# afombravo/2FAST2Q

Hardware: AMD Instinct MI355X
Metric: Mreads/sec matched (150 bp, 20 bp feature, m=1) (higher is better)
Workload: dtype u64 (2-bit packed bases) / u8 qualities

## Files before the change

2fast2q_amd/csrc/f2q_count_kernels.h:

```cpp
#pragma once

#define F2Q_HIST_MAX 24576u
#define F2Q_HIST_RANGE 38912u

__device__ __forceinline__ unsigned long long wave_sum(unsigned long long v)
{
    for (int o = 32; o > 0; o >>= 1) v += __shfl_down(v, o, 64);
    return v;
}

__device__ __forceinline__ void flush_stats(const Accum &acc, unsigned long long st[5], unsigned long long *lds8,
                                            unsigned long long *slab_row)
{
    const uint32_t lane = threadIdx.x & 63u;
    if (threadIdx.x < 8) lds8[threadIdx.x] = 0;
    __syncthreads();
    for (int k = 0; k < 5; k++) {
        unsigned long long v = wave_sum(st[k]);
        if (lane == 0 && v) atomicAdd(&lds8[k], v);
    }
    __syncthreads();
    if (threadIdx.x < 5) {
        unsigned long long v = lds8[threadIdx.x];
        if (slab_row) gpw(slab_row)[threadIdx.x] = v;
// ... 332 lines not shown
                    for (int r = 0; r < F2Q_MAXQROWS; r++)
                        if (r < g.nq) fixed4_qrow(g, r, qrow[r], bad);
                }
#pragma unroll
                for (int j = 0; j < 4; j++) {
                    if (res[j] != R_NEAR || bad[j]) continue;
                    key[j] |= fixed4_key(g, brow, j) << (2u * (uint32_t)L * npart[j]);
                    if (lv[j] & F2Q_LEN_FLAG) forced[j] |= fixed4_flags(g, qrow, j) << ((uint32_t)L * npart[j]);
                    npart[j]++;
                }
            }
#pragma unroll
            for (int j = 0; j < 4; j++) {
                if (res[j] == R_SLOW) {
                    unsigned long long st2[5] = {0, 0, 0, 0, 0};
                    const Accum acc2 = acc; const PackedBlock pb2 = pb;
                    multi_slow(runp, libp, &acc2, &pb2, tile, 4u * lane + (uint32_t)j, (int)(lv[j] & F2Q_LEN_MASK), st2);
#pragma unroll
                    for (int k = 0; k < 5; k++) st[k] += st2[k];
                    res[j] = R_SKIP;
                } else if (res[j] == R_NEAR) {
                    st[0]++;
                    if (npart[j] == 0u) { res[j] = R_QFAIL; st[4]++; }
                    else if (forced[j]) res[j] = (!do_near || __popc(forced[j]) > run.miss) ? R_NONALIGNED : R_FORCED;
                }
            }
            for (int k = W; k >= 1; k--) {
                bool mine[4]; bool any = false;
#pragma unroll
                for (int j = 0; j < 4; j++) { mine[j] = res[j] == R_NEAR && npart[j] == (uint32_t)k; any |= mine[j]; }
                if (__ballot(any) == 0ull) continue;
                const PackedGroup &pk = lib.mpk[k - 1];
                const PackedPiece ex = pk.exact;
                const uint32_t ib = pk.ib, exm = (1u << ex.bits) - 1u;
                const uint64_t imask = (1ull << ib) - 1ull;
                if (pk.len == 0u) continue;
                uint32_t s[4];
#pragma unroll
                for (int j = 0; j < 4; j++) s[j] = packed_start(key[j], ex.bits);
                while (mine[0] | mine[1] | mine[2] | mine[3]) {
                    uint64_t v0[4], v1[4];
#pragma unroll
                    for (int j = 0; j < 4; j++)
                        if (mine[j]) { const Slot2 pr = packed_pair(ptab, ex.off + s[j]); v0[j] = pr.a; v1[j] = pr.b; }
#pragma unroll
                    for (int j = 0; j < 4; j++) {
                        if (!mine[j]) continue;
                        if (v0[j] == KEY_EMPTY) mine[j] = false;
                        else if ((v0[j] >> ib) == key[j]) { mine[j] = false; res[j] = R_PERFECT; count_hit((uint32_t)(v0[j] & imask)); }
                        else if (v1[j] == KEY_EMPTY) mine[j] = false;
                        else if ((v1[j] >> ib) == key[j]) { mine[j] = false; res[j] = R_PERFECT; count_hit((uint32_t)(v1[j] & imask)); }
                        else s[j] = (s[j] + 2u) & exm;
                    }
                }
            }
            uint32_t npush = 0;
#pragma unroll
            for (int j = 0; j < 4; j++) {
                if (res[j] == R_NEAR) { if (do_near) npush++; else res[j] = R_NONALIGNED; }
                else if (res[j] == R_FORCED) npush++;
                st[1] += (res[j] == R_PERFECT); st[3] += (res[j] == R_NONALIGNED);
            }
            {
                const unsigned long long b0 = __ballot(npush & 1u), b1 = __ballot(npush & 2u), b2 = __ballot(npush & 4u);
                uint32_t at = q_tail + __builtin_amdgcn_mbcnt_hi((uint32_t)(b0 >> 32), __builtin_amdgcn_mbcnt_lo((uint32_t)b0, 0u))
                              + 2u * __builtin_amdgcn_mbcnt_hi((uint32_t)(b1 >> 32), __builtin_amdgcn_mbcnt_lo((uint32_t)b1, 0u))
                              + 4u * __builtin_amdgcn_mbcnt_hi((uint32_t)(b2 >> 32), __builtin_amdgcn_mbcnt_lo((uint32_t)b2, 0u));
                q_tail += (uint32_t)__popcll(b0) + 2u * (uint32_t)__popcll(b1) + 4u * (uint32_t)__popcll(b2);
#pragma unroll
                for (int j = 0; j < 4; j++)
                    if (res[j] == R_NEAR || res[j] == R_FORCED) {
                        queue[at % F2Q_V2_QCAP] = key[j] | ((unsigned long long)(npart[j] - 1u) << 62);
                        qforced[at % F2Q_V2_QCAP] = forced[j];
                        at++;
                    }
            }
        }
        if (do_near) drain(false);
    }
    if (do_near) drain(true);
    __shared__ unsigned long long st_lds[8];
    flush_stats(acc, st, st_lds, acc.stat_slab ? acc.stat_slab + (uint64_t)blockIdx.x * 8u : nullptr);
    if (USE_LDS) {
        __syncthreads();
        auto row = gpw(acc.slab) + (uint64_t)blockIdx.x * nf;
        for (uint32_t i = tid; i < nf; i += F2Q_V2_THREADS) row[i] = hist[i];
    }
}

#define F2Q_LT_THREADS 1024
#define F2Q_LT_WAVES (F2Q_LT_THREADS / 64)

__device__ __forceinline__ U2 lds_u2(const uint32_t *p)
{
    typedef uint32_t v2 __attribute__((ext_vector_type(2)));
    const v2 v = *reinterpret_cast<const v2 *>(p);
    return U2{v.x, v.y};
}

__device__ __forceinline__ uint32_t lt_count_add(uint32_t *cnt, uint32_t slot)
{
    return atomicAdd(&cnt[slot >> 1], 1u << ((slot & 1u) << 4));
}
__device__ __forceinline__ bool lt_count_passed(uint32_t old, uint32_t slot) { return ((old >> ((slot & 1u) << 4)) & 0xFFFFu) == 0x7FFFu; }
__device__ __forceinline__ void lt_count_handoff(uint32_t *cnt, uint32_t slot, const Accum &acc, const LtDesc &lt)
{
    atomicSub(&cnt[slot >> 1], 0x8000u << ((slot & 1u) << 4));
    acc_add(&acc.counts[gp(lt.feat_of)[slot]], 0x8000ull);
}
__device__ __forceinline__ void lt_count(uint32_t *cnt, uint32_t slot, const Accum &acc, const LtDesc &lt)
{
    if (lt_count_passed(lt_count_add(cnt, slot), slot)) lt_count_handoff(cnt, slot, acc, lt);
}

template <int NQ, int NB, bool NEAR, bool A20, bool MW = false>
__global__ __launch_bounds__(F2Q_LT_THREADS) void k_count_fixed4_lds(const RunDev *__restrict__ runp,
                                                                     const LibDev *__restrict__ libp, PackedBlock pb,
                                                                     Accum acc)
{
    extern __shared__ uint32_t lt_smem[];
    constexpr uint32_t NT = NEAR ? 2u : 1u;
    uint32_t *tg = lt_smem;
    uint32_t *cnt = lt_smem + NT * F2Q_LT_SLOTS;
    const RunDev &run = *runp;
    const LibDev &lib = *libp;
    LtDesc lt = lib.lt;
    if (A20) { lt.hb0 = 20u; lt.hb1 = 20u; lt.len = 20u; }
    const uint32_t nf = lib.n_features;
    const uint32_t tid = threadIdx.x, lane = tid & 63u;
    const uint32_t wave = (uint32_t)__builtin_amdgcn_readfirstlane((int)(tid >> 6));
    FixedGeom g = MW ? fixed_geom_at(0, run.n_iter * run.length, run.thr) : fixed_geom(run);
    if (A20) { g.L = 20; g.nq = 5; g.nb = 2; g.sh = 0; g.qm_first = 0x80808080u; g.qm_last = 0x80808080u; g.kmask = (1ull << 40) - 1ull; }
    const int need = g.st + g.L;
    uint32_t w_reads = 0, w_perfect = 0, w_imperfect = 0, w_qfail = 0;
    constexpr int QR = NQ ? NQ : F2Q_MAXQROWS, BR = NB ? NB : F2Q_MAXBROWS;
    constexpr bool PIPE = NQ != 0;

    struct Rows { U4 b[BR], q[QR]; uint32_t len01, len23; };
    const uint64_t q_stride = (uint64_t)pb.wq * F2Q_TILE, b_stride = (uint64_t)pb.wb * F2Q_TILE;
    const auto q_base = gp(pb.qual) + (uint64_t)g.qw0 * F2Q_TILE + 4u * lane;
    const auto b_base = gp(pb.bases) + (uint64_t)g.bw0 * F2Q_TILE + 4u * lane;
    const auto l_base = gp(pb.len) + 4u * lane;
    auto request_tile = [&](Rows &r, uint32_t t) {
        const auto qp = q_base + (uint64_t)t * q_stride;
        const auto bp = b_base + (uint64_t)t * b_stride;
#pragma unroll
        for (int i = 0; i < BR; i++) r.b[i] = ld_u4<true>(bp + (NB ? i : (i < g.nb ? i : g.nb - 1)) * F2Q_TILE);
#pragma unroll
        for (int i = 0; i < QR; i++) r.q[i] = ld_u4<true>(qp + (NQ ? i : (i < g.nq ? i : g.nq - 1)) * F2Q_TILE);
        typedef uint32_t v2 __attribute__((ext_vector_type(2)));
        const v2 lv = __builtin_nontemporal_load((const v2 F2Q_GLOBAL *)(l_base + (uint64_t)t * F2Q_TILE));
        r.len01 = lv.x; r.len23 = lv.y;
    };
    uint32_t pend_old[4] = {0, 0, 0, 0}, pend_slot[4] = {0, 0, 0, 0}, n_pend = 0;
    auto settle = [&]() {
        bool any = false;
#pragma unroll
        for (int k = 0; k < 4; k++)
            if ((uint32_t)k < n_pend) any |= lt_count_passed(pend_old[k], pend_slot[k]);
        if (any) {
#pragma unroll
            for (int k = 0; k < 4; k++)
                if ((uint32_t)k < n_pend && lt_count_passed(pend_old[k], pend_slot[k])) lt_count_handoff(cnt, pend_slot[k], acc, lt);
        }
        n_pend = 0;
    };
    auto decide_tile = [&](const Rows &r) {
        uint32_t bad[4] = {0, 0, 0, 0};
        bool part_fail[4] = {false, false, false, false};
        if (MW && g.add_hi) {
#pragma unroll
            for (int j = 0; j < 4; j++) {
                const int pv = mw_part_verdict(fixed4_failbits(g, r.q, j), run.n_iter, run.length);
                bad[j] = pv == 2 ? 1u : 0u; part_fail[j] = pv == 1;
            }
        } else if (g.add_hi) {
            if (A20) {
#pragma unroll
                for (int i = 0; i < QR; i++) {
#pragma unroll
                    for (int j = 0; j < 4; j++) {
                        const uint32_t w = u4get(r.q[i], j) & 0x7F7F7F7Fu;
                        bad[j] |= (w + g.add_lo) & ~(w + g.add_hi);
                    }
                }
#pragma unroll
                for (int j = 0; j < 4; j++) bad[j] &= 0x80808080u;
            } else {
#pragma unroll
                for (int i = 0; i < QR; i++)
                    if (NQ || i < g.nq) fixed4_qrow(g, i, r.q[i], bad);
            }
        }
        LtProbe0 p[4]; U2 e0[4], e1[4]; uint32_t klo[4], khi[4], forced[4]; bool cand[4];
#pragma unroll
        for (int j = 0; j < 4; j++) {
            const uint32_t l = ((j < 2 ? r.len01 : r.len23) >> (16 * (j & 1))) & 0xFFFFu;
            const bool live = l != F2Q_LEN_SKIP, qf = live && bad[j] != 0u;
            cand[j] = live && !qf && (int)(l & F2Q_LEN_MASK) >= need && !(MW && part_fail[j]);
            w_reads += (uint32_t)__popcll(__ballot(live));
            w_qfail += (uint32_t)__popcll(__ballot(qf));
            forced[j] = 0;
            if ((l & F2Q_LEN_FLAG) && cand[j]) forced[j] = fixed4_flags(g, r.q, j);
            uint64_t key = fixed4_key(g, r.b, j);
            if (MW && lt.mix) { key = mw_mix(key, lt.mix); if (forced[j]) forced[j] = mw_mix_mask(forced[j], lt.mix); }
            p[j] = lt_probe0(lt, key);
            e0[j] = lds_u2(tg + 2u * p[j].b0);
            e1[j] = lds_u2(tg + 2u * p[j].b1);
            klo[j] = (uint32_t)key; khi[j] = lt_rec_hi(key, forced[j]);
        }
        LtExact x[4];
#pragma unroll
        for (int j = 0; j < 4; j++) x[j] = lt_exact_stage(p[j], e0[j], e1[j], cand[j], forced[j]);
        settle();
#pragma unroll
        for (int j = 0; j < 4; j++) {
            pend_old[j] = 0;
            if (x[j].hit) pend_old[j] = lt_count_add(cnt, x[j].slot);
            pend_slot[j] = x[j].slot;
            w_perfect += (uint32_t)__popcll(__ballot(x[j].hit));
        }
        n_pend = 4;
        if (!NEAR) return;
        uint32_t pre[5], pos[4];
        pre[0] = 0;
#pragma unroll
        for (int j = 0; j < 4; j++) {
            const unsigned long long m = __ballot(x[j].batch);
            pos[j] = pre[j] + __builtin_amdgcn_mbcnt_hi((uint32_t)(m >> 32), __builtin_amdgcn_mbcnt_lo((uint32_t)m, 0u));
            pre[j + 1] = pre[j] + (uint32_t)__popcll(m);
        }
        for (uint32_t lo = 0; lo < pre[4]; lo += 64u) {
            const uint32_t at = lo + lane;
            uint32_t rlo = 0, rhi = 0;
#pragma unroll
            for (int j = 0; j < 4; j++) {
                if (!lt_batch_has(pre, j, lo)) continue;
                const bool send = x[j].batch && pos[j] - lo < 64u;
                const int to = (int)(4u * (send ? pos[j] - lo : lt_dump(pre, j, lo)));
                const uint32_t a = (uint32_t)__builtin_amdgcn_ds_permute(to, (int)klo[j]);
                const uint32_t b = (uint32_t)__builtin_amdgcn_ds_permute(to, (int)khi[j]);
                const bool mine = at >= pre[j] && at < pre[j + 1];
                rlo = mine ? a : rlo; rhi = mine ? b : rhi;
            }
            const bool valid = at < pre[4];
            const LtProbe q = lt_probe(lt, lt_rec_key(rlo, rhi));
            U2 e[4];
#pragma unroll
            for (int k = 0; k < 4; k++) e[k] = lds_u2(tg + (uint32_t)(k >> 1) * F2Q_LT_SLOTS + 2u * q.b[k]);
            const LtVerdict v = lt_decide<NEAR>(lt, q, e, lt_rec_forced(rhi), [&](uint32_t bk) { return lds_u2(tg + 2u * bk); });
            settle();
            const LtPred cm = LT_P(valid), perfect = v.perfect & cm, imperfect = v.imperfect & cm;
            pend_old[0] = 0;
            if (LT_TRUE(perfect | imperfect)) pend_old[0] = lt_count_add(cnt, v.slot);
            pend_slot[0] = v.slot;
            n_pend = 1;
            w_perfect += (uint32_t)__popcll(perfect);
            w_imperfect += (uint32_t)__popcll(imperfect);
        }
    };

    const uint32_t stride = gridDim.x * F2Q_LT_WAVES;
    uint32_t tile = blockIdx.x * F2Q_LT_WAVES + wave;
    const uint32_t last = pb.n_tiles - 1u;
    Rows ra, rb;
    if (PIPE && tile < pb.n_tiles) request_tile(ra, tile);
    {
        typedef uint32_t v4 __attribute__((ext_vector_type(4)));
        const v4 F2Q_GLOBAL *src = (const v4 F2Q_GLOBAL *)gp(lt.tags);
        v4 *dst = reinterpret_cast<v4 *>(tg);
        for (uint32_t i = tid; i < NT * F2Q_LT_SLOTS / 4u; i += F2Q_LT_THREADS) dst[i] = src[i];
        for (uint32_t i = tid; i < F2Q_LT_BUCKETS; i += F2Q_LT_THREADS) cnt[i] = 0;
    }
    __syncthreads();
    if (PIPE) {
        if (tile < pb.n_tiles) {
            for (;;) {
                __builtin_amdgcn_sched_barrier(0);
                request_tile(rb, min(tile + stride, last));
                __builtin_amdgcn_sched_barrier(0);
                decide_tile(ra);
                tile += stride;
                if (tile >= pb.n_tiles) break;
                __builtin_amdgcn_sched_barrier(0);
                request_tile(ra, min(tile + stride, last));
                __builtin_amdgcn_sched_barrier(0);
                decide_tile(rb);
                tile += stride;
                if (tile >= pb.n_tiles) break;
            }
        }
    } else {
        for (; tile < pb.n_tiles; tile += stride) { Rows r; request_tile(r, tile); decide_tile(r); }
    }
    settle();
    __syncthreads();
    {
        auto row = gpw(acc.slab) + (uint64_t)blockIdx.x * nf;
        for (uint32_t i = tid; i < nf; i += F2Q_LT_THREADS) {
            const uint32_t s = gp(lt.slot_of)[i];
            row[i] = (cnt[s >> 1] >> ((s & 1u) << 4)) & 0xFFFFu;
        }
    }
    __syncthreads();
    const bool l0 = lane == 0;
    unsigned long long stv[5] = {l0 ? w_reads : 0u, l0 ? w_perfect : 0u, l0 ? w_imperfect : 0u,
                                 l0 ? w_reads - w_perfect - w_imperfect - w_qfail : 0u, l0 ? w_qfail : 0u};
    flush_stats(acc, stv, reinterpret_cast<unsigned long long *>(lt_smem), acc.stat_slab + (uint64_t)blockIdx.x * 8u);
}

__global__ __launch_bounds__(F2Q_V2_THREADS) void k_extract_fixed4(const RunDev *__restrict__ runp, EcDev ec, PackedBlock pb,
                                                                    Accum acc, uint64_t read_base)
{
    const RunDev &run = *runp;
    const uint32_t tid = threadIdx.x, lane = tid & 63u, wave = tid >> 6;
    const FixedGeom g = fixed_geom(run);
    unsigned long long st[5] = {0, 0, 0, 0, 0};
    uint32_t n_new = 0;
    for (uint32_t base = blockIdx.x * F2Q_V2_WAVES; base < pb.n_tiles; base += gridDim.x * F2Q_V2_WAVES) {
        const uint32_t tile = base + wave;
        if (tile >= pb.n_tiles) continue;
        U4 brow[F2Q_MAXBROWS], qrow[F2Q_MAXQROWS];
        const auto qp = gp(pb.qual) + (uint64_t)tile * pb.wq * F2Q_TILE + 4u * lane;
        const auto bp = gp(pb.bases) + (uint64_t)tile * pb.wb * F2Q_TILE + 4u * lane;
#pragma unroll
        for (int r = 0; r < F2Q_MAXBROWS; r++) {
            uint32_t row = (uint32_t)g.bw0 + (uint32_t)(r < g.nb ? r : (g.nb > 0 ? g.nb - 1 : 0));
            row = row < pb.wb ? row : pb.wb - 1u;
            brow[r] = ld_u4<true>(bp + (uint64_t)row * F2Q_TILE);
        }
#pragma unroll
        for (int r = 0; r < F2Q_MAXQROWS; r++) {
            const uint32_t want = (uint32_t)g.qw0 + (uint32_t)(r < g.nq ? r : (g.nq > 0 ? g.nq - 1 : 0));
            const uint32_t row = want < pb.wq ? want : pb.wq - 1u;
            qrow[r] = want < pb.wq ? ld_u4<true>(qp + (uint64_t)row * F2Q_TILE) : U4{0, 0, 0, 0};
        }
        uint32_t len01 = 0, len23 = 0;
        if (pb.len) {
            typedef uint32_t v2 __attribute__((ext_vector_type(2)));
            v2 lv = *(const v2 F2Q_GLOBAL *)(gp(pb.len) + (uint64_t)tile * F2Q_TILE + 4u * lane);
            len01 = lv.x; len23 = lv.y;
        }
        uint32_t bad[4] = {0, 0, 0, 0};
        if (g.add_hi) {
#pragma unroll
            for (int r = 0; r < F2Q_MAXQROWS; r++)
                if (r < g.nq) fixed4_qrow(g, r, qrow[r], bad);
        }
#pragma unroll
        for (int j = 0; j < 4; j++) {
            const uint32_t l = pb.len ? (((j < 2 ? len01 : len23) >> (16 * (j & 1))) & 0xFFFFu) : pb.rmax;
            if (l == F2Q_LEN_SKIP) continue;
            st[0]++;
            if (bad[j]) { st[4]++; continue; }
            const uint64_t slot = (uint64_t)tile * F2Q_TILE + 4u * lane + (uint32_t)j;
            n_new += ec64_insert_word(ec, fixed4_ec_word(g, brow, qrow, j, l), read_base + pb.first_index + (pb.index ? (uint64_t)gp(pb.index)[slot] : slot));
            st[1]++;
        }
    }
    ec64_report_new(ec, n_new);
    __shared__ unsigned long long st_lds[8];
    flush_stats(acc, st, st_lds, nullptr);
}

#define F2Q_AN_THREADS 256
#define F2Q_AN_WAVES (F2Q_AN_THREADS / 64)
#define F2Q_AN_QCAP 512u

__device__ __noinline__ void anchor_slow(const RunDev *run, const LibDev *lib, const EcDev *ec, const Accum *acc,
                                         const PackedBlock *pb, uint32_t tile, uint32_t slot, int r,
                                         unsigned long long read_index, unsigned long long *st, bool lower = false)
{
    uint8_t seq[F2Q_ANCHOR_MAXLEN], qual[F2Q_ANCHOR_MAXLEN];
    const uint32_t nw = pb->planar_nw;
    const auto bp = gp(pb->bases) + (uint64_t)tile * pb->wb * F2Q_TILE + slot;
    const auto qp = gp(pb->qual) + (uint64_t)tile * pb->wq * F2Q_TILE + slot;
    if (r > F2Q_ANCHOR_MAXLEN) r = F2Q_ANCHOR_MAXLEN;
    for (int i = 0; i < r; i++) {
        const uint32_t lo = bp[(uint64_t)(i >> 5) * F2Q_TILE], hi = bp[(uint64_t)(nw + (i >> 5)) * F2Q_TILE];
        seq[i] = (uint8_t)"ACGT"[((lo >> (i & 31)) & 1u) | (((hi >> (i & 31)) & 1u) << 1)];
        qual[i] = (uint8_t)((qp[(uint64_t)planar_qword((uint32_t)i) * F2Q_TILE] >> (8 * planar_qbyte((uint32_t)i))) & 0xFFu);
        if (qual[i] & 0x80u) { seq[i] = lower ? (uint8_t)(seq[i] | 0x20u) : (uint8_t)'N'; qual[i] &= 0x7Fu; }
    }
    general_read<const uint8_t *>(*run, *lib, *ec, *acc, seq, r, qual, r, read_index, st);
}

template <int NW, int KB, bool EC, bool USE_LDS, bool SAMEQ>
__global__ __launch_bounds__(F2Q_AN_THREADS) void k_count_anchor(const RunDev *__restrict__ runp,
                                                                  const LibDev *__restrict__ libp, EcDev ec,
                                                                  PackedBlock pb, Accum acc, uint64_t read_base)
{
    constexpr int NQW = 8 * NW;
    extern __shared__ unsigned long long smem64[];
    unsigned long long *queue = smem64 + (threadIdx.x >> 6) * F2Q_AN_QCAP;
    uint32_t *qforced = reinterpret_cast<uint32_t *>(smem64 + F2Q_AN_WAVES * F2Q_AN_QCAP) + (threadIdx.x >> 6) * F2Q_AN_QCAP;
    uint32_t *hist = reinterpret_cast<uint32_t *>(smem64 + F2Q_AN_WAVES * F2Q_AN_QCAP) + F2Q_AN_WAVES * F2Q_AN_QCAP;
    const RunDev &run = *runp;
    const LibDev &lib = *libp;
    const uint32_t nf = lib.n_features;
    const uint32_t tid = threadIdx.x, lane = tid & 63u;
    if (USE_LDS && !EC) for (uint32_t i = tid; i < nf; i += F2Q_AN_THREADS) hist[i] = 0;
    __syncthreads();
    uint32_t q_head = 0, q_tail = 0;
    const bool do_near = run.miss > 0;
    const int pk_len = (int)lib.pk.len;
    const uint32_t ah_w = phred_add_hi(run.thr), ah_u = phred_add_hi(run.thr_up), ah_d = phred_add_hi(run.thr_down);
    unsigned long long st[5] = {0, 0, 0, 0, 0};
    uint32_t n_new = 0;
#ifdef F2Q_STAMP
    unsigned long long tp[6] = {0, 0, 0, 0, 0, 0}, t0_, t1_;
#define STAMP(i) do { __builtin_amdgcn_sched_barrier(0); t1_ = __builtin_amdgcn_s_memtime(); __builtin_amdgcn_s_waitcnt(0xC07F); tp[i] += t1_ - t0_; t0_ = t1_; __builtin_amdgcn_sched_barrier(0); } while (0)
#else
#define STAMP(i) do {} while (0)
#endif

    auto count_hit = [&](uint32_t idx) {
        if (USE_LDS) atomicAdd(&hist[idx], 1u);
        else acc_add(&acc.counts[idx], 1ull);
    };

    uint32_t nLO[NW], nHI[NW], nQ[NQW], nl = F2Q_LEN_SKIP;
    auto request_tile = [&](uint32_t t) {
        const auto bpn = gp(pb.bases) + (uint64_t)t * pb.wb * F2Q_TILE + tid;
        const auto qpn = gp(pb.qual) + (uint64_t)t * pb.wq * F2Q_TILE + tid;
        nl = pb.len ? gp(pb.len)[(uint64_t)t * F2Q_TILE + tid] : pb.rmax;
#pragma unroll
        for (int w = 0; w < NW; w++) {
            nLO[w] = __builtin_nontemporal_load(bpn + (uint64_t)w * F2Q_TILE);
            nHI[w] = __builtin_nontemporal_load(bpn + (uint64_t)(NW + w) * F2Q_TILE);
        }
#pragma unroll
        for (int i = 0; i < NQW; i++) nQ[i] = __builtin_nontemporal_load(qpn + (uint64_t)i * F2Q_TILE);
    };
    if (blockIdx.x < pb.n_tiles) request_tile(blockIdx.x);
    for (uint32_t tile = blockIdx.x; tile < pb.n_tiles; tile += gridDim.x) {
#ifdef F2Q_STAMP
        __builtin_amdgcn_sched_barrier(0); t0_ = __builtin_amdgcn_s_memtime(); __builtin_amdgcn_s_waitcnt(0xC07F);
#endif
        const uint32_t l = nl;
        uint32_t LO[NW], HI[NW], Q[NQW];
#pragma unroll
        for (int w = 0; w < NW; w++) { LO[w] = nLO[w]; HI[w] = nHI[w]; }
#pragma unroll
        for (int i = 0; i < NQW; i++) Q[i] = nQ[i];
        __builtin_amdgcn_sched_barrier(0);
        if (tile + gridDim.x < pb.n_tiles) request_tile(tile + gridDim.x);
// ... 939 lines not shown
```

2fast2q_amd/csrc/f2q_device.h:

```cpp
#pragma once
#include <stdint.h>

#ifndef F2Q_HD
#ifdef __HIPCC__
#define F2Q_HD __host__ __device__ __forceinline__
#else
#define F2Q_HD inline
#endif
#endif

#define F2Q_DEV_MAX_ITER 16
#define F2Q_ANCHOR_MAX 128
#define F2Q_MAX_PIECES 8
#define F2Q_REG_MAXLEN 31
#define F2Q_TILE 256
#define F2Q_LEN_SKIP 0xFFFFu
#define F2Q_LEN_FLAG 0x8000u
#define F2Q_LEN_CASE 0x4000u
#define F2Q_LEN_MASK 0x3FFFu

namespace f2q {

#if defined(__HIP_DEVICE_COMPILE__)
#define F2Q_GLOBAL __attribute__((address_space(1)))
// ... 1190 lines not shown
F2Q_HD uint32_t lt_near1(const LtDesc &lt, const LtProbe &q, const U2 (&e)[4], uint32_t forced, uint32_t &hit, uint32_t &hitw)
{
    const uint32_t l0 = lt.hb0 >> 1;
    const uint32_t f0 = forced & ((1u << l0) - 1u), f1 = forced >> l0;
    uint32_t nf = 0, keep0 = ~0u, keep1 = ~0u;
    if (forced) {
#if defined(__HIP_DEVICE_COMPILE__)
        nf = (uint32_t)__popc(forced);
#else
        nf = (uint32_t)__builtin_popcount(forced);
#endif
        const uint32_t s0 = spread16(f0), s1 = spread16(f1);
        keep0 = ~(s0 | (s0 << 1)); keep1 = ~(s1 | (s1 << 1));
    }
    uint32_t n = 0;
    hit = 0; hitw = 0;
    const uint32_t m0 = (1u << lt.hb0) - 1u, m1 = (1u << lt.hb1) - 1u;
#pragma unroll
    for (int k = 0; k < 4; k++) {
        const bool t1 = k >= 2;
        const bool open = t1 ? (f1 == 0u) : (f0 == 0u);
        const uint32_t ob = t1 ? lt.hb0 : lt.hb1, om = t1 ? m0 : m1, oq = t1 ? q.h0 : q.h1, keep = t1 ? keep0 : keep1;
#pragma unroll
        for (int i = 0; i < 2; i++) {
            const uint32_t w = i ? e[k].y : e[k].x;
            const bool same = (w >> ob) == q.cmp[k];
            const uint32_t d = ham2_32(((w ^ oq) & om) & keep) + nf;
            const bool c = open & same & (d == 1u);
            n += (uint32_t)c;
            hit = c ? (((uint32_t)t1 << 31) | (2u * q.b[k] + (uint32_t)i)) : hit;
            hitw = c ? w : hitw;
        }
    }
    return n;
}
template <class RD>
F2Q_HD uint32_t lt_slot_of_t1(const LtDesc &lt, const LtProbe &q, uint32_t hitw, RD rd)
{
    const uint32_t fh0 = hitw & ((1u << lt.hb0) - 1u);
    uint32_t b0, c0, b1, c1;
    lt_hash(fh0, lt.hb0, lt.hb1, 0, b0, c0); lt_hash(fh0, lt.hb0, lt.hb1, 1, b1, c1);
    const U2 e0 = rd(b0), e1 = rd(b1);
    const uint32_t w0 = lt_tag(c0, q.h1, lt.hb1), w1 = lt_tag(c1, q.h1, lt.hb1);
    const bool a1 = e0.y == w0, hit0 = (e0.x == w0) | a1, b1y = e1.y == w1;
    return hit0 ? 2u * b0 + (uint32_t)a1 : 2u * b1 + (uint32_t)b1y;
}

#if defined(__HIP_DEVICE_COMPILE__)
typedef unsigned long long LtPred;
#define LT_P(c) __ballot(c)
#define LT_TRUE(p) __builtin_amdgcn_inverse_ballot_w64(p)
#define LT_NOT(p) (~(p))
#else
typedef bool LtPred;
#define LT_P(c) (c)
#define LT_TRUE(p) (p)
#define LT_NOT(p) (!(p))
#endif
#define LT_SEL(p, a, b) (LT_TRUE(p) ? (a) : (b))

struct LtSide { uint32_t x, slot; LtPred any, multi, first; };
F2Q_HD LtSide lt_side(uint32_t want0, uint32_t want1, uint32_t limit, uint32_t b0, uint32_t b1, const U2 &e0, const U2 &e1)
{
    const uint32_t x0 = e0.x ^ want0, x1 = e0.y ^ want0, x2 = e1.x ^ want1, x3 = e1.y ^ want1;
    const LtPred s0 = LT_P(x0 < limit), s1 = LT_P(x1 < limit), s2 = LT_P(x2 < limit), s3 = LT_P(x3 < limit);
    LtSide r;
    r.x = LT_SEL(s0, x0, LT_SEL(s1, x1, LT_SEL(s2, x2, x3)));
    r.first = s0 | s1;
    r.any = r.first | s2 | s3;
    r.multi = (s0 & (s1 | s2 | s3)) | (s1 & (s2 | s3)) | (s2 & s3);
    const LtPred odd = (LT_NOT(s0) & s1) | (LT_NOT(r.first) & LT_NOT(s2));
    r.slot = 2u * LT_SEL(r.first, b0, b1) + (LT_TRUE(odd) ? 1u : 0u);
    return r;
}
struct LtVerdict { LtPred perfect, imperfect, via1; uint32_t slot; };
template <bool NEAR, bool T1SLOT = false, class RD>
F2Q_HD LtVerdict lt_decide(const LtDesc &lt, const LtProbe &q, const U2 (&e)[4], uint32_t forced, RD rd0)
{
    const uint32_t w0 = lt_tag(q.cmp[0], q.h1, lt.hb1), w1 = lt_tag(q.cmp[1], q.h1, lt.hb1);
    const LtSide a = lt_side(w0, w1, 1u << lt.hb1, q.b[0], q.b[1], e[0], e[1]);
    LtSide b = a;
    uint32_t w2 = 0, w3 = 0;
    const LtPred unforced = LT_P(forced == 0u);
    LtPred fast = LT_NOT(a.multi);
    if (!NEAR) fast = fast & unforced;
    LtPred perfect = unforced & fast & a.any & LT_P(a.x == 0u), near = perfect & LT_NOT(perfect);
    LtPred through1 = near;
    uint32_t slot = a.slot;
    if (NEAR) {
        w2 = lt_tag(q.cmp[2], q.h0, lt.hb0); w3 = lt_tag(q.cmp[3], q.h0, lt.hb0);
        b = lt_side(w2, w3, 1u << lt.hb0, q.b[2], q.b[3], e[2], e[3]);
        fast = fast & LT_NOT(b.multi);
        perfect = perfect & fast;
        const LtPred c0 = a.any & LT_P(ham2_32(a.x) == 1u), c1 = b.any & LT_P(ham2_32(b.x) == 1u);
        near = unforced & fast & LT_NOT(perfect) & (c0 ^ c1);
        LtPred via1 = near & c1;
#if defined(__HIP_DEVICE_COMPILE__)
        const bool some_forced = LT_NOT(unforced) != 0ull;
#else
        const bool some_forced = forced != 0u;
#endif
        if (some_forced) {
            const uint32_t l0 = lt.hb0 >> 1;
            const uint32_t p = forced ? lt_ctz(forced) : 0u;
            const bool in0 = p < l0;
            const uint32_t keep = ~(3u << (2u * (in0 ? p : p - l0)));
            const uint32_t xs = in0 ? b.x : a.x;
            const LtPred one = LT_P((forced & (forced - 1u)) == 0u);
            const LtPred g = LT_NOT(unforced) & one & fast & LT_P((xs & keep) == 0u) & LT_P(in0 ? LT_TRUE(b.any) : LT_TRUE(a.any));
            near = near | g;
            via1 = via1 | (g & LT_P(in0));
        }
        if (T1SLOT) { slot = LT_SEL(via1, b.slot, slot); through1 = via1; }
        else if (LT_TRUE(via1)) slot = lt_slot_of_t1(lt, q, b.x ^ LT_SEL(b.first, w2, w3), rd0);
    }
    int sres = 0;
    bool sv1 = false;
    if (!LT_TRUE(fast)) {
        sres = R_NONALIGNED;
        const int ex = forced == 0u ? lt_exact(lt, q, e[0], e[1]) : -1;
        if (ex >= 0) { sres = R_PERFECT; slot = (uint32_t)ex; }
#if defined(__HIP_DEVICE_COMPILE__)
        else if (NEAR && __popc(forced) <= 1) {
#else
        else if (NEAR && __builtin_popcount(forced) <= 1) {
#endif
            uint32_t hit = 0, hitw = 0;
            if (lt_near1(lt, q, e, forced, hit, hitw) == 1u) {
                sres = R_IMPERFECT;
                if (T1SLOT) { slot = hit & 0x7FFFFFFFu; sv1 = (hit >> 31) != 0u; }
                else slot = (hit >> 31) ? lt_slot_of_t1(lt, q, hitw, rd0) : (hit & 0x7FFFFFFFu);
            }
        }
    }
    LtVerdict v;
    v.perfect = perfect | LT_P(sres == R_PERFECT);
    v.imperfect = near | LT_P(sres == R_IMPERFECT);
    v.via1 = through1 | LT_P(sv1);
    v.slot = slot;
    return v;
}

struct LtProbe0 { uint32_t b0, b1, w0, w1; };
F2Q_HD LtProbe0 lt_probe0(const LtDesc &lt, uint64_t key)
{
    const uint32_t h0 = (uint32_t)key & ((1u << lt.hb0) - 1u), h1 = (uint32_t)(key >> lt.hb0);
    LtProbe0 p;
    uint32_t c0, c1;
    lt_hash(h0, lt.hb0, lt.hb1, 0, p.b0, c0);
    lt_hash(h0, lt.hb0, lt.hb1, 1, p.b1, c1);
    p.w0 = lt_tag(c0, h1, lt.hb1); p.w1 = lt_tag(c1, h1, lt.hb1);
    return p;
}
struct LtExact { bool hit, batch; uint32_t slot; };
F2Q_HD LtExact lt_exact_stage(const LtProbe0 &p, const U2 &e0, const U2 &e1, bool cand, uint32_t forced)
{
    const bool a0 = e0.x == p.w0, a1 = e0.y == p.w0, b0 = e1.x == p.w1, b1 = e1.y == p.w1;
    LtExact r;
    r.hit = cand && forced == 0u && (a0 | a1 | b0 | b1);
    r.batch = cand && !r.hit;
    r.slot = (a0 | a1) ? 2u * p.b0 + (uint32_t)a1 : 2u * p.b1 + (uint32_t)b1;
    return r;
}
F2Q_HD uint32_t lt_rec_hi(uint64_t key, uint32_t forced) { return (uint32_t)(key >> 32) | (forced << 10); }
F2Q_HD uint64_t lt_rec_key(uint32_t lo, uint32_t hi) { return ((uint64_t)(hi & 0x3FFu) << 32) | lo; }
F2Q_HD uint32_t lt_rec_forced(uint32_t hi) { return hi >> 10; }
F2Q_HD uint32_t lt_dump(const uint32_t (&pre)[5], int j, uint32_t lo)
{
    const uint32_t s = (pre[j] > lo ? pre[j] : lo) - lo, e = pre[j + 1] - lo < 64u ? pre[j + 1] - lo : 64u;
    return e < 64u ? e : (s ? s - 1u : 0u);
}
F2Q_HD bool lt_batch_has(const uint32_t (&pre)[5], int j, uint32_t lo) { return pre[j] < lo + 64u && pre[j + 1] > lo; }

F2Q_HD uint32_t funnel_shr(uint32_t hi, uint32_t lo, int sh)
{
#if defined(__HIP_DEVICE_COMPILE__)
    return __builtin_amdgcn_alignbit(hi, lo, (uint32_t)sh);
#else
    return sh ? ((lo >> sh) | (hi << (32 - sh))) : lo;
#endif
}
F2Q_HD int ctz32(uint32_t x)
{
#if defined(__HIP_DEVICE_COMPILE__)
    return __ffs((int)x) - 1;
#else
    return __builtin_ctz(x);
#endif
}
F2Q_HD uint32_t range_mask32(int lo, int hi)
{
    lo = lo < 0 ? 0 : lo; hi = hi > 32 ? 32 : hi;
    if (hi <= lo) return 0u;
    uint32_t upper = hi >= 32 ? ~0u : ((1u << hi) - 1u);
    return upper & (lo >= 32 ? 0u : (~0u << lo));
}

template <int NW, int KB>
F2Q_HD void anchor_step(const uint32_t (&P)[NW], int j, uint32_t (&cnt)[KB > 0 ? KB : 1][NW], uint32_t (&ovf)[NW])
{
#pragma unroll
    for (int w = 0; w < NW; w++) {
        uint32_t x = funnel_shr(w + 1 < NW ? P[w + 1] : ~0u, P[w], j);
        if (KB == 0) ovf[w] |= x;
        else {
#pragma unroll
            for (int b = 0; b < KB; b++) { uint32_t c = cnt[b][w] & x; cnt[b][w] ^= x; x = c; }
            ovf[w] |= x;
        }
    }
}

template <int NW, int KB>
F2Q_HD void anchor_step2(const uint32_t (&P)[NW], int j1, int j2, uint32_t (&cnt)[KB > 0 ? KB : 1][NW], uint32_t (&ovf)[NW])
{
#pragma unroll
    for (int w = 0; w < NW; w++) {
        const uint32_t up = w + 1 < NW ? P[w + 1] : ~0u;
        const uint32_t x1 = funnel_shr(up, P[w], j1), x2 = funnel_shr(up, P[w], j2);
        if (KB == 0) ovf[w] |= x1 | x2;
        else {
            const uint32_t c0 = cnt[0][w];
#if defined(__HIP_DEVICE_COMPILE__)
            uint32_t x = __builtin_amdgcn_bitop3_b32(c0, x1, x2, 0xE8);
            cnt[0][w] = __builtin_amdgcn_bitop3_b32(c0, x1, x2, 0x96);
#else
            uint32_t x = (c0 & x1) | (c0 & x2) | (x1 & x2);
            cnt[0][w] = c0 ^ x1 ^ x2;
#endif
#pragma unroll
            for (int b = 1; b < KB; b++) { uint32_t c = cnt[b][w] & x; cnt[b][w] ^= x; x = c; }
            ovf[w] |= x;
        }
    }
}
template <int NW, int KB>
F2Q_HD void anchor_steps(const uint32_t (&P)[NW], uint32_t m, uint32_t (&cnt)[KB > 0 ? KB : 1][NW], uint32_t (&ovf)[NW])
{
    while (m & (m - 1u)) {
        const int j1 = ctz32(m); m &= m - 1u;
        const int j2 = ctz32(m); m &= m - 1u;
        anchor_step2<NW, KB>(P, j1, j2, cnt, ovf);
    }
    if (m) anchor_step<NW, KB>(P, ctz32(m), cnt, ovf);
}

template <int NW, int KB>
F2Q_HD void anchor_compare(const uint32_t (&cnt)[KB > 0 ? KB : 1][NW], const uint32_t (&ovf)[NW], int k, uint32_t (&hit)[NW])
{
#pragma unroll
    for (int w = 0; w < NW; w++) {
        uint32_t gt = 0, eq = ~0u;
#pragma unroll
        for (int b = KB - 1; b >= 0; b--) {
            if ((k >> b) & 1) eq &= cnt[b][w];
            else { gt |= eq & cnt[b][w]; eq &= ~cnt[b][w]; }
        }
        hit[w] = ~gt & ~ovf[w];
    }
}

template <int NW, int KBU, int KBD>
F2Q_HD void anchor_hits2p(const RunDev &run, const uint32_t *up_pos, const uint32_t *down_pos,
                          const uint32_t (&LO)[NW], const uint32_t (&HI)[NW], const uint32_t (&FLG)[NW],
                          uint32_t (&hu)[NW], uint32_t (&hd)[NW])
{
    uint32_t cu[KBU > 0 ? KBU : 1][NW], ou[NW], cd[KBD > 0 ? KBD : 1][NW], od[NW];
#pragma unroll
    for (int w = 0; w < NW; w++) {
        ou[w] = 0; od[w] = 0;
#pragma unroll
        for (int b = 0; b < (KBU > 0 ? KBU : 1); b++) cu[b][w] = 0;
#pragma unroll
        for (int b = 0; b < (KBD > 0 ? KBD : 1); b++) cd[b][w] = 0;
    }
#pragma unroll
    for (int c = 0; c < 4; c++) {
        const uint32_t la = (c & 1) ? ~0u : 0u, ha = (c & 2) ? ~0u : 0u;
        uint32_t P[NW];
#pragma unroll
        for (int w = 0; w < NW; w++) P[w] = (LO[w] ^ la) | (HI[w] ^ ha) | FLG[w];
        if (run.has_up) anchor_steps<NW, KBU>(P, up_pos[c], cu, ou);
        if (run.has_down) anchor_steps<NW, KBD>(P, down_pos[c], cd, od);
    }
    anchor_compare<NW, KBU>(cu, ou, run.msu, hu);
    anchor_compare<NW, KBD>(cd, od, run.msd, hd);
}
template <int NW, int KBU, int KBD>
F2Q_HD void anchor_hits2(const RunDev &run, const uint32_t (&LO)[NW], const uint32_t (&HI)[NW], const uint32_t (&FLG)[NW],
                         uint32_t (&hu)[NW], uint32_t (&hd)[NW])
{
    anchor_hits2p<NW, KBU, KBD>(run, run.up_pos, run.down_pos, LO, HI, FLG, hu, hd);
}

template <int NW>
F2Q_HD int first_hit(const uint32_t (&hit)[NW], int from, int to)
{
    int pos = -1;
#pragma unroll
    for (int w = NW - 1; w >= 0; w--) {
        const uint32_t m = hit[w] & range_mask32(from - 32 * w, to + 1 - 32 * w);
        if (m) pos = 32 * w + ctz32(m);
    }
    return pos;
}

template <int NW>
F2Q_HD bool any_in_range(const uint32_t (&F)[NW], int a, int b)
{
    uint32_t acc = 0;
#pragma unroll
    for (int w = 0; w < NW; w++) acc |= F[w] & range_mask32(a - 32 * w, b - 32 * w);
    return acc != 0;
}
// ... 358 lines not shown
```

Before: 176,500.

## Split tile decision into extract and settle stages with single-buffer prefetch

Splits the per-tile work into an extract stage (quality check, key hashing, LDS tag loads) and a settle stage (exact match, counter atomics, near-match batch). The loop now issues the next tile's global loads between the two stages, so the LDS reads can complete while the prefetch is in flight, and it keeps one Rows buffer instead of two. The pending-counter overflow check becomes a packed bitwise test on the 16-bit halves, and the atomics use a precomputed bucket and increment. The A20 path also runs even when add_hi is zero, substituting add_lo. Register pressure from the hoisted probe state and the reordered schedule could reduce occupancy.

```diff
diff --git a/2fast2q_amd/csrc/f2q_count_kernels.h b/2fast2q_amd/csrc/f2q_count_kernels.h
--- a/2fast2q_amd/csrc/f2q_count_kernels.h
+++ b/2fast2q_amd/csrc/f2q_count_kernels.h
@@ -508,20 +508,25 @@
         const v2 lv = __builtin_nontemporal_load((const v2 F2Q_GLOBAL *)(l_base + (uint64_t)t * F2Q_TILE));
         r.len01 = lv.x; r.len23 = lv.y;
     };
-    uint32_t pend_old[4] = {0, 0, 0, 0}, pend_slot[4] = {0, 0, 0, 0}, n_pend = 0;
+    uint32_t pend_old[4] = {0, 0, 0, 0}, pend_at[4] = {0, 0, 0, 0}, pend_inc[4] = {1, 1, 1, 1}, n_pend = 0;
     auto settle = [&]() {
-        bool any = false;
-#pragma unroll
-        for (int k = 0; k < 4; k++)
-            if ((uint32_t)k < n_pend) any |= lt_count_passed(pend_old[k], pend_slot[k]);
-        if (any) {
-#pragma unroll
-            for (int k = 0; k < 4; k++)
-                if ((uint32_t)k < n_pend && lt_count_passed(pend_old[k], pend_slot[k])) lt_count_handoff(cnt, pend_slot[k], acc, lt);
+        uint32_t f = (pend_old[0] + 0x00010001u) & ~pend_old[0];
+        if (n_pend > 1u) {
+#pragma unroll
+            for (int k = 1; k < 4; k++) f |= (pend_old[k] + 0x00010001u) & ~pend_old[k];
+        }
+        if ((f & 0x80008000u) != 0u) {
+#pragma unroll
+            for (int k = 0; k < 4; k++) {
+                const uint32_t slot = 2u * pend_at[k] + (pend_inc[k] >> 16);
+                if ((uint32_t)k < n_pend && lt_count_passed(pend_old[k], slot)) lt_count_handoff(cnt, slot, acc, lt);
+            }
         }
         n_pend = 0;
     };
-    auto decide_tile = [&](const Rows &r) {
+    LtProbe0 p[4]; U2 e0[4], e1[4]; uint32_t klo[4], khi[4], forced[4]; bool cand[4];
+    const uint32_t a20_hi = g.add_hi ? g.add_hi : g.add_lo;
+    auto extract = [&](const Rows &r) {
         uint32_t bad[4] = {0, 0, 0, 0};
         bool part_fail[4] = {false, false, false, false};
         if (MW && g.add_hi) {
@@ -530,14 +535,14 @@
                 const int pv = mw_part_verdict(fixed4_failbits(g, r.q, j), run.n_iter, run.length);
                 bad[j] = pv == 2 ? 1u : 0u; part_fail[j] = pv == 1;
             }
-        } else if (g.add_hi) {
+        } else if (A20 || g.add_hi) {
             if (A20) {
 #pragma unroll
                 for (int i = 0; i < QR; i++) {
 #pragma unroll
                     for (int j = 0; j < 4; j++) {
                         const uint32_t w = u4get(r.q[i], j) & 0x7F7F7F7Fu;
-                        bad[j] |= (w + g.add_lo) & ~(w + g.add_hi);
+                        bad[j] |= (w + g.add_lo) & ~(w + a20_hi);
                     }
                 }
 #pragma unroll
@@ -548,14 +553,14 @@
                     if (NQ || i < g.nq) fixed4_qrow(g, i, r.q[i], bad);
             }
         }
-        LtProbe0 p[4]; U2 e0[4], e1[4]; uint32_t klo[4], khi[4], forced[4]; bool cand[4];
+        uint32_t t_reads = 0, t_qfail = 0;
 #pragma unroll
         for (int j = 0; j < 4; j++) {
             const uint32_t l = ((j < 2 ? r.len01 : r.len23) >> (16 * (j & 1))) & 0xFFFFu;
             const bool live = l != F2Q_LEN_SKIP, qf = live && bad[j] != 0u;
             cand[j] = live && !qf && (int)(l & F2Q_LEN_MASK) >= need && !(MW && part_fail[j]);
-            w_reads += (uint32_t)__popcll(__ballot(live));
-            w_qfail += (uint32_t)__popcll(__ballot(qf));
+            t_reads += (uint32_t)__popcll(__ballot(live));
+            t_qfail += (uint32_t)__popcll(__ballot(qf));
             forced[j] = 0;
             if ((l & F2Q_LEN_FLAG) && cand[j]) forced[j] = fixed4_flags(g, r.q, j);
             uint64_t key = fixed4_key(g, r.b, j);
@@ -564,7 +569,12 @@
             e0[j] = lds_u2(tg + 2u * p[j].b0);
             e1[j] = lds_u2(tg + 2u * p[j].b1);
             klo[j] = (uint32_t)key; khi[j] = lt_rec_hi(key, forced[j]);
-        }
+            asm volatile("" : "+v"(klo[j]), "+v"(khi[j]), "+v"(p[j].w0), "+v"(p[j].w1));
+        }
+        w_reads += t_reads; w_qfail += t_qfail;
+        asm volatile("" : "+s"(w_reads), "+s"(w_qfail));
+    };
+    auto settle_tile = [&]() {
         LtExact x[4];
 #pragma unroll
         for (int j = 0; j < 4; j++) x[j] = lt_exact_stage(p[j], e0[j], e1[j], cand[j], forced[j]);
@@ -572,8 +582,8 @@
 #pragma unroll
         for (int j = 0; j < 4; j++) {
             pend_old[j] = 0;
-            if (x[j].hit) pend_old[j] = lt_count_add(cnt, x[j].slot);
-            pend_slot[j] = x[j].slot;
+            pend_at[j] = x[j].bucket; pend_inc[j] = x[j].odd ? 0x10000u : 1u;
+            if (x[j].hit) pend_old[j] = atomicAdd(&cnt[pend_at[j]], pend_inc[j]);
             w_perfect += (uint32_t)__popcll(__ballot(x[j].hit));
         }
         n_pend = 4;
@@ -608,8 +618,8 @@
             settle();
             const LtPred cm = LT_P(valid), perfect = v.perfect & cm, imperfect = v.imperfect & cm;
             pend_old[0] = 0;
-            if (LT_TRUE(perfect | imperfect)) pend_old[0] = lt_count_add(cnt, v.slot);
-            pend_slot[0] = v.slot;
+            pend_at[0] = v.slot >> 1; pend_inc[0] = 1u << ((v.slot & 1u) << 4);
+            if (LT_TRUE(perfect | imperfect)) pend_old[0] = atomicAdd(&cnt[pend_at[0]], pend_inc[0]);
             n_pend = 1;
             w_perfect += (uint32_t)__popcll(perfect);
             w_imperfect += (uint32_t)__popcll(imperfect);
@@ -619,8 +629,8 @@
     const uint32_t stride = gridDim.x * F2Q_LT_WAVES;
     uint32_t tile = blockIdx.x * F2Q_LT_WAVES + wave;
     const uint32_t last = pb.n_tiles - 1u;
-    Rows ra, rb;
-    if (PIPE && tile < pb.n_tiles) request_tile(ra, tile);
+    Rows rows;
+    if (PIPE && tile < pb.n_tiles) request_tile(rows, tile);
     {
         typedef uint32_t v4 __attribute__((ext_vector_type(4)));
         const v4 F2Q_GLOBAL *src = (const v4 F2Q_GLOBAL *)gp(lt.tags);
@@ -630,24 +640,15 @@
     }
     __syncthreads();
     if (PIPE) {
-        if (tile < pb.n_tiles) {
-            for (;;) {
-                __builtin_amdgcn_sched_barrier(0);
-                request_tile(rb, min(tile + stride, last));
-                __builtin_amdgcn_sched_barrier(0);
-                decide_tile(ra);
-                tile += stride;
-                if (tile >= pb.n_tiles) break;
-                __builtin_amdgcn_sched_barrier(0);
-                request_tile(ra, min(tile + stride, last));
-                __builtin_amdgcn_sched_barrier(0);
-                decide_tile(rb);
-                tile += stride;
-                if (tile >= pb.n_tiles) break;
-            }
+        for (; tile < pb.n_tiles; tile += stride) {
+            extract(rows);
+            __builtin_amdgcn_sched_barrier(0);
+            request_tile(rows, min(tile + stride, last));
+            __builtin_amdgcn_sched_barrier(0);
+            settle_tile();
         }
     } else {
-        for (; tile < pb.n_tiles; tile += stride) { Rows r; request_tile(r, tile); decide_tile(r); }
+        for (; tile < pb.n_tiles; tile += stride) { request_tile(rows, tile); extract(rows); settle_tile(); }
     }
     settle();
     __syncthreads();
diff --git a/2fast2q_amd/csrc/f2q_device.h b/2fast2q_amd/csrc/f2q_device.h
--- a/2fast2q_amd/csrc/f2q_device.h
+++ b/2fast2q_amd/csrc/f2q_device.h
@@ -1366,14 +1366,15 @@
     p.w0 = lt_tag(c0, h1, lt.hb1); p.w1 = lt_tag(c1, h1, lt.hb1);
     return p;
 }
-struct LtExact { bool hit, batch; uint32_t slot; };
+struct LtExact { bool hit, batch, odd; uint32_t slot, bucket; };
 F2Q_HD LtExact lt_exact_stage(const LtProbe0 &p, const U2 &e0, const U2 &e1, bool cand, uint32_t forced)
 {
     const bool a0 = e0.x == p.w0, a1 = e0.y == p.w0, b0 = e1.x == p.w1, b1 = e1.y == p.w1;
     LtExact r;
     r.hit = cand && forced == 0u && (a0 | a1 | b0 | b1);
     r.batch = cand && !r.hit;
-    r.slot = (a0 | a1) ? 2u * p.b0 + (uint32_t)a1 : 2u * p.b1 + (uint32_t)b1;
+    r.bucket = (a0 | a1) ? p.b0 : p.b1; r.odd = (a0 | a1) ? a1 : b1;
+    r.slot = 2u * r.bucket + (uint32_t)r.odd;
     return r;
 }
 F2Q_HD uint32_t lt_rec_hi(uint64_t key, uint32_t forced) { return (uint32_t)(key >> 32) | (forced << 10); }
```

Measured after the change: 179,700, median of 6. 1.8% higher.
